# rodluger/starry_process

Measured on AMD Instinct MI355X. Metric: log_likelihood evals/sec (ydeg=15, K=1000), higher is better.
Workload: dtype f64

## Files before the change

### include/starry_process_amd.h

```cpp
#ifndef STARRY_PROCESS_AMD_H
#define STARRY_PROCESS_AMD_H

#include <stdint.h>

#ifdef __cplusplus
extern "C" {
#endif

typedef struct sp_handle sp_handle;

typedef enum {
  SP_OK = 0,
  SP_ERR_INVALID = -1,
  SP_ERR_HIP = -2,
  SP_ERR_NO_DEVICE = -3,
  SP_ERR_STATE = -4,
  SP_ERR_ALLOC = -5,
  SP_ERR_COMM = -6
} sp_status;

#define SP_STAR_NOT_PD 1u
#define SP_STAR_ZMAX 2u
#define SP_STAR_NAN 4u
#define SP_STAR_STALE_PLAN 8u
// ... 185 lines not shown
                         double *dnodes_da_host, double *dweights_da_host, double *dnodes_db_host,
                         double *dweights_db_host);

int sp_ylm_moments_quadrature(sp_handle *h, const double *vecs_host, int mv, int first_is_col,
                              const double *phi_host, const double *w_host, int P, int Q, double g,
                              double sqrt_n, double epsy, double epsy15, double *mean_dev,
                              double *cov_dev, void *stream);
int sp_ylm_moments_quadrature_grad(sp_handle *h, const double *s_host, const double *ds_dr_host,
                                   const double *phi_host, const double *w_host, const double *dphi_host,
                                   const double *dw_host, int P, int Q, double g, double sqrt_n, double epsy,
                                   double epsy15, double *mean_dev, double *cov_dev, double *dmean_dev,
                                   double *dcov_dev, void *stream);

int sp_profile_begin(sp_handle *h, int max_launches);
int sp_profile_end(sp_handle *h, long *launches, double *total_ms, double *flops);
int sp_profile_kind(sp_handle *h, int kind, long *launches, double *total_ms, double *flops);
int sp_profile_kind_ex(sp_handle *h, int kind, long *launches, double *total_ms, double *flops, double *flops_padded);
int sp_profile_begin_kinds(sp_handle *h, int max_launches, unsigned kind_mask);

int sp_set_defer_norm(sp_handle *h, int on);

int sp_set_lazy_cov(sp_handle *h, int on);

int sp_allgather_lnlike(sp_handle *h, void *nccl_comm, const double *local_dev, int count,
                        double *all_dev, void *stream);

int sp_debug_set_look_ahead(sp_handle *h, int on);
int sp_debug_set_panel_layout(sp_handle *h, int layout, int fuse_reduce);
int sp_debug_panel2_trace(long long *out);
int sp_debug_panel2_chain(long long *out);
int sp_debug_set_syrk128_from(int blocks);
int sp_debug_set_syrk_symdiag(int on);
int sp_debug_set_small_k(int on);
int sp_debug_asm_chunks(int ntr, int nchunk, int *start_host);

#ifdef __cplusplus
}
#endif
#endif
```

### starry_process_amd/_lib.py

```python
import ctypes
import os

import numpy as np

_HERE = os.path.dirname(os.path.abspath(__file__))
LIB_PATH = os.path.join(_HERE, "libsp_hip.so")
if os.environ.get("SP_LIB_VARIANT"):
    LIB_PATH = os.path.join(_HERE, "libsp_hip_%s.so" % os.environ["SP_LIB_VARIANT"])

c_double_p = ctypes.POINTER(ctypes.c_double)
c_int32_p = ctypes.POINTER(ctypes.c_int32)
c_void_p = ctypes.c_void_p


class sp_star(ctypes.Structure):

    _fields_ = [
        ("period", ctypes.c_double),
        ("inc", ctypes.c_double),
        ("tau", ctypes.c_double),
        ("baseline_var", ctypes.c_double),
        ("baseline_mean", ctypes.c_double),
        ("data_var", ctypes.c_double),
        ("table", ctypes.c_int32),
# ... 58 lines not shown
    "sp_ylm_conditional_workspace_bytes": (ctypes.c_size_t, [_V, _I, _I]),
    "sp_ylm_conditional_batched": (_I, [_V, _I, _I, _V, _V, _V, _V, _V, _V, _V, _V, _V, _V, _V, _V, _V]),
    "sp_ylm_conditional_whitened": (_I, [_V, _I, _I, _V, _V, _V, _V, _V, _V, _V, _V, _V, _V]),
    "sp_alpha_beta": (_I, [_D, _I, c_double_p, c_double_p, c_double_p, c_double_p]),
    "sp_set_marginal_constants": (_I, [_V, _V, _V]),
    "sp_set_ylm_moments": (_I, [_V, _V, _V]),
    "sp_set_ylm_moments_dev": (_I, [_V, _V, _V, _V]),
    "sp_get_polar_moments": (_I, [_V, _V, _V]),
    "sp_ylm_moments_quadrature": (_I, [_V, _V, _I, _I, _V, _V, _I, _I, _D, _D, _D, _D,
                                       _V, _V, _V]),
    "sp_ylm_moments_quadrature_grad": (_I, [_V, _V, _V, _V, _V, _V, _V, _I, _I, _D, _D, _D, _D,
                                            _V, _V, _V, _V, _V]),
    "sp_debug_panel2_trace": (_I, [_V]),
    "sp_debug_panel2_chain": (_I, [_V]),
    "sp_debug_asm_chunks": (_I, [_I, _I, _V]),
    "sp_debug_set_syrk128_from": (_I, [_I]),
    "sp_debug_set_small_k": (_I, [_I]),
    "sp_debug_set_syrk_symdiag": (_I, [_I]),
    "sp_debug_set_look_ahead": (_I, [_V, _I]),
    "sp_debug_set_panel_layout": (_I, [_V, _I, _I]),
    "sp_profile_kind": (_I, [_V, _I, ctypes.POINTER(ctypes.c_long), c_double_p, c_double_p]),
    "sp_profile_kind_ex": (_I, [_V, _I, ctypes.POINTER(ctypes.c_long), c_double_p, c_double_p, c_double_p]),
    "sp_set_lazy_cov": (_I, [_V, _I]),
    "sp_set_defer_norm": (_I, [_V, _I]),
    "sp_profile_begin_kinds": (_I, [_V, _I, ctypes.c_uint]),
    "sp_profile_begin": (_I, [_V, _I]),
    "sp_profile_end": (_I, [_V, ctypes.POINTER(ctypes.c_long), c_double_p, c_double_p]),
    "sp_kernel_table": (_I, [_V, _V, _I, _I, _V, _V, _V, _V]),
    "sp_cov_marginal_batched": (
        _I, [_V, _I, _I, _V, _V, _I, _V, _V, _I, _I, _I, _V, _L, _L, _V, _V]),
    "sp_design_matrix": (_I, [_V, _I, _I, _V, _V, _V, _V, _V]),
    "sp_cov_conditional_batched": (
        _I, [_V, _I, _I, _V, _V, _V, _I, _I, _I, _V, _L, _L, _V, _V, _V]),
    "sp_cho_factor": (_I, [_V, _V, _I, _L, _L, _I, _V, _V]),
    "sp_cho_solve": (_I, [_V, _V, _I, _L, _L, _V, _I, _I, _V]),
    "sp_tri_solve": (_I, [_V, _V, _I, _L, _L, _V, _I, _I, _I, _V]),
    "sp_solve_rev": (_I, [_V, _V, _I, _L, _L, _V, _V, _I, _I, _I, _V, _V, _V]),
    "sp_cholesky_rev": (_I, [_V, _V, _I, _L, _L, _V, _I, _V, _V]),
    "sp_lnlike_workspace_bytes": (_L, [_V, _I, _I, _I]),
    "sp_lnlike_ensemble": (
        _I, [_V, _I, _I, _I, _V, _V, _V, _V, _I, _I, _V, _V, _V, _I, _I, _I, _D,
             _V, _V, _V, _V]),
    "sp_cholesky_lnlike_batched": (_I, [_V, _I, _I, _I, _V, _V, _V, _V, _V, _V]),
    "sp_plan_data": (_I, [_V, _I, _I, _I, _V, _V, _V, _V, _I, _I, _V, _V, ctypes.POINTER(_V)]),
    "sp_plan_destroy": (None, [_V]),
    "sp_plan_replicate": (_I, [_V, _V, _I, _V, ctypes.POINTER(_V)]),
# ... 76 lines not shown
```

### starry_process_amd/csrc/sp_api.hip

```cpp
#include <algorithm>
#include <cmath>
#include <cstdio>
#include <cstdlib>
#include <dlfcn.h>
#include <cstring>
#include <new>

#include "sp_internal.h"
#include "sp_cov.h"

int sp_launch_kernel_table(sp_handle *h, const double *rta1_dev, int ntab,
                           int covpts, const double *xp_dev, double *tab_dev,
                           double *meanvar_dev, hipStream_t st, int nsets = 0, const double *ez_dev = nullptr,
                           const double *Ez_dev = nullptr);
int sp_launch_theta(int S, int K, const double *t, const sp_star *stars,
                    double *theta, hipStream_t st, int32_t *info = nullptr,
                    uint32_t *status = nullptr, const double *tab = nullptr, int covpts = 0,
                    double *ptab = nullptr);
int sp_launch_spline_index(int K, const double *theta, double dx, long long *out,
                           hipStream_t st);
int sp_launch_rowsum(int S, int K, const double *theta, const double *t,
                     const sp_star *stars, int covpts, const double *tab,
                     const double *meanvar, const double *xp, int temporal,
                     const double *raw, double *rowsum, hipStream_t st);
// ... 11 lines not shown
                       int lazy_nfull = 0);
int sp_launch_assemble_sums(int S, int K, int M, int Kp, const double *theta, const double *t,
                            const sp_star *stars, int covpts, const double *ptab, const double *meanvar,
                            int temporal, const double *flux, double *sys, hipStream_t st, double *part,
                            int lazy_nfull, int *nflat);
int sp_launch_defer_finish(int S, int K, int M, int Kp, const sp_star *stars, const double *meanvar,
                           const double *condmean, int order, double zmax, const double *part,
                           const double *diag, const double *flux, double *sys, void *coef, double *rscal,
                           uint32_t *status, hipStream_t st, int nflat = 0);
int sp_launch_assemble_planned(int S, int K, int M, int Kp, const PlanDev &plan, const double *t,
                               const sp_star *stars, int covpts, const double *tab, const double *meanvar,
                               int temporal, const double *flux, const double *diag, double *sys, int nfull,
                               int ncolw, int order, double zmax, void *coef, double *rscal, double *ptab, int32_t *info,
                               uint32_t *status, hipStream_t st, double *img, long lts, int fuse0, double *rid, int dfrom);
int sp_launch_cholesky_systems(sp_handle *h, double *sys, int S, int K, int Kp,
                               int32_t *info, double *invL, hipStream_t st);
bool sp_small_k_serves(int K, int M, int covpts, bool has_diag);
static int g_small_k = -1;
static bool sp_small_k_on() {
  if (g_small_k >= 0) return g_small_k != 0;
  static const bool env = !(getenv("SP_SMALL_K") && atoi(getenv("SP_SMALL_K")) == 0);
  return env;
}
int sp_launch_small_lnlike(int S, int K, int M, const PlanDev &plan, const double *t, const sp_star *stars, int covpts,
                           const double *tab, const double *meanvar, int temporal, const double *flux, const double *diag,
                           int order, double zmax, double *lnlike, uint32_t *status_out, hipStream_t st);
int sp_launch_cond_system(const double *B1, const double *A, int N, int Kr, int S, int K, int M, int Kp,
                          const double *t, const sp_star *stars, int temporal, const void *coef,
                          const double *diag, const double *flux, double *sys, double *part,
                          hipStream_t st);
int sp_launch_cholesky_groups(sp_handle *h, int ngroups, const sp_chol_group *grp, int K,
                              int Kp);
int sp_launch_lnlike_reduce(const double *sys, int S, int K, int M, int Kp,
                            const int32_t *info, double *lnlike, uint32_t *status,
                            hipStream_t st, uint32_t *status_out = nullptr,
                            const sp_star *stars = nullptr, const void *defer_coef = nullptr,
                            const double *rscal = nullptr, int dvec = 0);
int sp_launch_pad_in(const double *A, int K, long lda, long strideA, double *sys,
                     int Kp, int M, const double *resid, int S, hipStream_t st, int ident = 0,
                     int32_t *nonfinite = nullptr);
int sp_launch_pad_out(const double *sys, int Kp, double *A, int K, long lda,
                      long strideA, const int32_t *info, int S, hipStream_t st);
int sp_launch_cho_solve(const double *L, int K, long ldl, long strideL, double *B,
                        int nrhs, int batch, hipStream_t st);
int sp_launch_ylm_gram(int S, int K, int N, const double *A, const double *flux, const double *diag,
                       const sp_star *stars, int whitened, const double *sinv, const double *sinvmu, double *Bt,
// ... 716 lines not shown
    ms += dt;
    fl += h->prof_fl[i / 2];
    flp += h->prof_flp[i / 2];
    n += h->prof_n[i / 2];
  }
  if (launches) *launches = n;
  if (total_ms) *total_ms = ms;
  if (flops) *flops = fl;
  if (flops_padded) *flops_padded = flp;
  return SP_OK;
}

int sp_profile_end(sp_handle *h, long *launches, double *total_ms, double *flops) {
  return sp_profile_kind(h, SP_PROF_SYRK, launches, total_ms, flops);
}

int sp_set_lazy_cov(sp_handle *h, int on) {
  if (h && h->device < 0) return SP_ERR_NO_DEVICE;
  if (!h) return SP_ERR_INVALID;
  h->lazy_cov = on ? 1 : 0;
  return SP_OK;
}

int sp_set_defer_norm(sp_handle *h, int on) {
  if (h && h->device < 0) return SP_ERR_NO_DEVICE;
  if (!h || (on != 0 && on != 1)) return SP_ERR_INVALID;
  h->defer_norm = on;
  return SP_OK;
}

int sp_debug_set_small_k(int on) {
  g_small_k = on < 0 ? -1 : (on ? 1 : 0);
  return SP_OK;
}

int sp_debug_set_look_ahead(sp_handle *h, int on) {
  if (!h) return SP_ERR_INVALID;
  h->look_ahead = on ? 1 : 0;
  return SP_OK;
}

int sp_debug_set_panel_layout(sp_handle *h, int layout, int fuse_reduce) {
  if (!h) return SP_ERR_INVALID;
  h->panel_layout = layout ? 1 : 0;
  h->fuse_reduce = fuse_reduce ? 1 : 0;
  return SP_OK;
// ... 356 lines not shown

int sp_lnlike_ensemble_planned(sp_handle *h, const sp_plan *plan, const double *t_dev, const double *flux_dev,
                               const double *diag_dev, const sp_star *stars_dev, const double *tab_dev,
                               const double *meanvar_dev, int norm_order, double zmax, void *workspace_dev,
                               double *lnlike_dev, uint32_t *status_dev, void *stream) {
  if (h && h->device < 0) return SP_ERR_NO_DEVICE;
  if (!h || !plan || !stars_dev || !tab_dev || !meanvar_dev || !workspace_dev || !lnlike_dev ||
      norm_order < 0 || norm_order > SP_NORM_MAXORDER)
    return SP_ERR_INVALID;
  if (plan->device != h->device) return SP_ERR_INVALID;
  if (!t_dev && !flux_dev && !diag_dev) {
    t_dev = plan->t;
    flux_dev = plan->flux;
    diag_dev = plan->diag;
  } else if (t_dev != plan->t || flux_dev != plan->flux || diag_dev != plan->diag) {
    return SP_ERR_INVALID;
  }
  const int S = plan->S, K = plan->K, M = plan->M, covpts = plan->covpts, temporal = plan->temporal;
  if (h->xp_covpts != covpts) return SP_ERR_STATE;
  hipStream_t st = (hipStream_t)stream;
  if (sp_small_k_on() && sp_small_k_serves(K, M, covpts, diag_dev != nullptr))
    return sp_launch_small_lnlike(S, K, M, plan->dev, t_dev, stars_dev, covpts, tab_dev, meanvar_dev, temporal, flux_dev,
                                  diag_dev, norm_order, zmax, lnlike_dev, status_dev, st);
  Layout L = make_layout(h, S, K, M, true);
  void *ws = workspace_dev;
  double *ptab = 4 * (size_t)(covpts + 4) > (size_t)L.Kr * L.N ? nullptr : at<double>(ws, L.A);
  int lazy_nfull = 0, ncolw = 0, no_panels = 0;
  static const bool riding_env = !(getenv("SP_PLAN_RIDING_LAZY") && atoi(getenv("SP_PLAN_RIDING_LAZY")) == 0);
  bool riding = false;
  const int nrid = M + (diag_dev ? 2 : 1);
  double *rid = at<double>(ws, L.B1);
  if (h->lazy_cov && ptab && K / SP_NB >= 2 && 4 * (covpts + 4) + 64 <= SP_TILE_LDS_MIN) {
    riding = riding_env && ((size_t)nrid + 1) * K <= (size_t)L.Kr * L.N;
    lazy_nfull = riding ? L.Kp / SP_NB : K / SP_NB;
    static const bool panel_lazy = !(getenv("SP_PLAN_PANEL_LAZY") && atoi(getenv("SP_PLAN_PANEL_LAZY")) == 0);
    if (temporal != SP_TEMPORAL_NONE || !panel_lazy) {
      static const bool tl = !(getenv("SP_PLAN_TEMPORAL_LAZY") && atoi(getenv("SP_PLAN_TEMPORAL_LAZY")) == 0);
      ncolw = sp_superpanel_width(h, K);
      no_panels = 1;
      if ((!tl && temporal != SP_TEMPORAL_NONE) || ncolw * SP_NB >= K) lazy_nfull = ncolw = no_panels = 0;
    }
  }
  static const bool dlazy_env = !(getenv("SP_PLAN_DIAG_LAZY") && atoi(getenv("SP_PLAN_DIAG_LAZY")) == 0);
  const int ntr = L.Kp / SP_NB, wsp = sp_superpanel_width(h, K), nsteps = (K + SP_NB - 1) / SP_NB;
  int dlazy = 0, dfrom = ntr;
  if (dlazy_env && riding && lazy_nfull == ntr && wsp * SP_NB < K && sp_syrk_can_form_diag(ntr - wsp) &&
// ... 1 lines not shown
    const int last = wsp < nsteps - 1 ? wsp : nsteps - 1;
    dlazy = 2;
    dfrom = last + 1;
  }
  static const bool fuse0_env = !(getenv("SP_PLAN_FUSE0") && atoi(getenv("SP_PLAN_FUSE0")) == 0);
  const int fuse0 = (fuse0_env && K >= SP_NB) ? 1 : 0;
  int rc = sp_launch_assemble_planned(S, K, M, L.Kp, plan->dev, t_dev, stars_dev, covpts, tab_dev, meanvar_dev, temporal,
                                      flux_dev, diag_dev, at<double>(ws, L.sys), lazy_nfull, ncolw, norm_order, zmax,
                                      at<double>(ws, L.coef), at<double>(ws, L.rscal), ptab, at<int32_t>(ws, L.info),
                                      at<uint32_t>(ws, L.status), st, at<double>(ws, L.invL), sp_lt_stride(L.Kp), fuse0,
                                      riding ? rid : nullptr, dfrom);
  if (rc) return rc;
  const bool fused_reduce = sp_panel_fuses_reduce(h, K, L.Kp);
  sp_chol_group G{at<double>(ws, L.sys), at<int32_t>(ws, L.info), at<double>(ws, L.invL), S, st, LazyCov{}, SpReduceArgs{}};
  if (fused_reduce)
    G.red = SpReduceArgs{lnlike_dev, at<uint32_t>(ws, L.status), status_dev, stars_dev, (const void *)at<double>(ws, L.coef),
                         at<double>(ws, L.rscal), diag_dev ? 1 : 0, K, M, K + M + (diag_dev ? 2 : 1)};
  G.block0_done = fuse0 != 0;
  (void)dlazy;
  if (lazy_nfull)
    G.lazy = LazyCov{plan->dev.theta, t_dev, stars_dev, ptab, K, covpts, temporal, lazy_nfull, 0, 0, no_panels ? 0 : 1,
                     no_panels, riding ? rid : nullptr, riding ? nrid : 0, dlazy, plan->dev.inorder};
  if ((rc = sp_launch_cholesky_groups(h, 1, &G, K, L.Kp))) return rc;
  if (!fused_reduce) return lnlike_finish(L, ws, K, M, lnlike_dev, status_dev, st, stars_dev, true, diag_dev != nullptr);
  return SP_OK;
}

int sp_gemm_nt(sp_handle *h, const double *A_dev, long lda, long strideA, const double *B_dev,
               long ldb, long strideB, double *C_dev, long ldc, long strideC, int M, int N,
               int K, double alpha, int beta, int lower_only, int batch, void *stream) {
  if (h && h->device < 0) return SP_ERR_NO_DEVICE;
  if (!h || !A_dev || !B_dev || !C_dev || M < 0 || N < 0 || K < 0 || batch < 0 || lda < K ||
      ldb < K || ldc < N || (beta != 0 && beta != 1))
    return SP_ERR_INVALID;
  return sp_launch_gemm_nt(A_dev, lda, strideA, B_dev, ldb, strideB, C_dev, ldc, strideC, M, N, K,
                           alpha, beta, lower_only, batch, (hipStream_t)stream);
}

int sp_gp_condition(sp_handle *h, int K, int Ks, const double *Ktt_dev, const double *Kst_dev,
                    double *Kss_dev, const double *r_dev, double *mu_dev, int32_t *info_dev,
                    void *stream) {
  if (h && h->device < 0) return SP_ERR_NO_DEVICE;
  if (!h || K < 1 || Ks < 1 || !Ktt_dev || !Kst_dev || !Kss_dev || !r_dev || !mu_dev)
    return SP_ERR_INVALID;
  hipStream_t st = (hipStream_t)stream;
  const int M = Ks + 1, Kp = sp_roundup(K + M, SP_NB);
  SpCarve c;
  const size_t osys = c.take(sizeof(double) * (size_t)Kp * Kp), ores = c.take(sizeof(double) * (size_t)M * K),
// ... 293 lines not shown
```

### starry_process_amd/csrc/sp_host.cpp

```cpp
#include <cmath>
#include <cstring>

#include "sp_internal.h"

namespace {

inline int nidx(int l, int m) { return l * l + l + m; }

inline void mono_mul_acc(double *acc, int l1, int m1, int l2, int m2, double v) {
  const bool z1 = ((l1 + m1) & 1) != 0, z2 = ((l2 + m2) & 1) != 0;
  const int l = l1 + l2, m = m1 + m2;
  if (z1 && z2) {
    acc[nidx(l - 2, m)] += v;
    acc[nidx(l, m - 2)] += -v;
    acc[nidx(l, m + 2)] += -v;
  } else {
    acc[nidx(l, m)] += v;
  }
}

void times_z(int deg, const double *p, double *out, int nout) {
  for (int i = 0; i < nout; ++i) out[i] = 0.0;
  for (int l = 0; l <= deg; ++l)
    for (int m = -l; m <= l; ++m) {
// ... 293 lines not shown
  return SP_OK;
}

int sp_alpha_beta(double z, int order, double *alpha, double *beta,
                  double *dalpha_dz, double *dbeta_dz) {
  if (order < 0) return SP_ERR_INVALID;
  double fac = 1.0, a = 0.0, b = 0.0, da = 0.0, db = 0.0, df = 0.0;
  for (int n = 0; n <= order; ++n) {
    da += df;
    db += 2 * n * df;
    df = (2 * n + 3) * (df * z + fac);
    a += fac;
    b += 2 * n * fac;
    fac *= z * (2 * n + 3);
  }
  if (alpha) *alpha = a;
  if (beta) *beta = b;
  if (dalpha_dz) *dalpha_dz = da;
  if (dbeta_dz) *dbeta_dz = db;
  return SP_OK;
}

int sp_version(void) { return 100; }

const char *sp_strerror(int status) {
  switch (status) {
    case SP_OK: return "ok";
    case SP_ERR_INVALID: return "invalid argument";
    case SP_ERR_HIP: return "HIP runtime error";
    case SP_ERR_NO_DEVICE: return "no usable gfx950 device";
    case SP_ERR_STATE: return "constants or Ylm moments not set";
    case SP_ERR_ALLOC: return "allocation failed";
    case SP_ERR_COMM: return "RCCL not loaded in this process, or the collective failed";
    default: return "unknown status";
  }
}

}

namespace {

double hyp2f1_series(double a, double b, double c, double z) {
  double term = a * b * z / c;
  double dtermdb = a * z / c, dtermdc = -term / c;
  double value = 1.0 + term, dfdb = dtermdb, dfdc = dtermdc;
  int n = 1;
// ... 227 lines not shown
```

### starry_process_amd/csrc/sp_internal.h

```cpp
#ifndef SP_INTERNAL_H
#define SP_INTERNAL_H

#include <hip/hip_runtime.h>
#include <stdint.h>
#include <vector>

#include "../../include/starry_process_amd.h"

#define SP_WAVE 64
#define SP_MAX_YDEG 30
#define SP_MAX_UDEG 4
#define SP_NORM_MAXORDER 64

#define SP_NB 64

struct SpScratch {
  void *ptr = nullptr;
  size_t bytes = 0;
};

struct sp_handle {
  int ydeg = 0, udeg = 0, N = 0, NWIG = 0, device = 0;
  std::vector<int32_t> l_of, m_of, mirror, m0, blk;
  std::vector<double> rT;
// ... 20 lines not shown
  SpScratch tab_scratch;
  bool table_attr_done = false;
  SpScratch big;
  struct CsSlot {
    double *host = nullptr;
    double *dev = nullptr;
    size_t cap = 0;
    hipEvent_t done = nullptr;
    bool used = false;
  };
  std::vector<CsSlot> cs_ring;
  int cs_next = 0;
  int superpanel = 0;
  int groups = 1;
  int ncu = 256;
  int look_ahead = 1;
  int panel_layout = 1;
  int fuse_reduce = 1;
  std::vector<hipStream_t> gstream;
  std::vector<hipEvent_t> gdone;
  hipEvent_t gfork = nullptr;
  int defer_norm = 1;
  int lazy_cov = 1;
  bool prof_on = false;
  unsigned prof_mask = 1u;
  std::vector<hipEvent_t> prof_ev;
  std::vector<int> prof_kind;
  std::vector<double> prof_fl;
  std::vector<double> prof_flp;
  std::vector<int> prof_n;
  size_t prof_used = 0;
};

enum {
  SP_PROF_SYRK = 0, SP_PROF_CHAIN = 2, SP_PROF_PANELS = 4, SP_PROF_PANEL_LAUNCH = 5, SP_PROF_NKINDS = 6
};

struct SpProfScope {
  sp_handle *h;
  hipStream_t st;
  bool on;
  size_t idx;
  SpProfScope(sp_handle *h_, hipStream_t st_, int kind, double flops, int launches = 1, double flops_padded = -1.0)
      : h(h_), st(st_), on(false), idx(0) {
    if (!h || !h->prof_on || !((h->prof_mask >> kind) & 1u) || h->prof_used + 2 > h->prof_ev.size()) return;
    idx = h->prof_used;
    h->prof_used += 2;
    h->prof_kind[idx / 2] = kind;
    h->prof_fl[idx / 2] = flops;
    h->prof_flp[idx / 2] = flops_padded < 0.0 ? flops : flops_padded;
    h->prof_n[idx / 2] = launches;
    if (hipEventRecord(h->prof_ev[idx], st) != hipSuccess) {
      h->prof_n[idx / 2] = 0;
      h->prof_fl[idx / 2] = 0.0;
      h->prof_flp[idx / 2] = 0.0;
      h->prof_kind[idx / 2] = -1;
      return;
    }
// ... 83 lines not shown
  int tr0, tc0;
  int c0lazy;
  int no_panels;
  const double *rid;
  int nrid;
  int dlazy;
  const double *inorder;
};

int sp_syrk_can_form_diag(int nb);

struct SpCoef {
  double c1;
  double zab;
  double za;
  double z;
  double gpmean;
  double m;
  double mu;
  double d1;
};
static_assert(sizeof(SpCoef) == 64, "8 doubles per star (Layout::coef)");

struct PlanDev {
  const double *theta;
  const double *wbar;
  const double *sflux;
  const double *sdv;
  const double *key;
  const double *inorder;
};
struct sp_plan {
  int device, S, K, M, covpts, temporal, has_diag;
  void *buf;
  size_t bytes;
  PlanDev dev;
  const double *t, *flux, *diag;
  int nrep;
};

#define SP_RSCAL_HEAD 3
struct SpReduceArgs {
  double *lnlike;
  uint32_t *status, *status_out;
  const sp_star *stars;
  const void *coef;
  const double *rscal;
  int dvec;
  int K, M;
  int live_rows;
};

struct sp_chol_group {
  double *sys;
  int32_t *info;
  double *invL;
  int S;
  hipStream_t st;
  LazyCov lazy;
  SpReduceArgs red;
  int tri0 = -1;
// ... 57 lines not shown
```

### starry_process_amd/csrc/sp_plan.hip

```cpp
#include <new>

#include "sp_internal.h"
#include "sp_cov.h"

int sp_launch_theta(int S, int K, const double *t, const sp_star *stars, double *theta, hipStream_t st,
                    int32_t *info = nullptr, uint32_t *status = nullptr, const double *tab = nullptr,
                    int covpts = 0, double *ptab = nullptr);

namespace {

template <int TK>
__global__ __launch_bounds__(256) void plan_wbar_kernel(
    int K, const double *__restrict__ theta, const double *__restrict__ t, const sp_star *__restrict__ stars,
    int covpts, double *__restrict__ partial) {
  extern __shared__ __attribute__((aligned(16))) double bins[];
  const int s = blockIdx.y, np = covpts + 4, tid = threadIdx.x, wave = tid >> 6;
  for (int k = tid; k < 4 * np; k += 256) bins[k] = 0.0;
  __syncthreads();
  const int tile = blockIdx.x;
  int ta = (int)((sqrtf(8.0f * tile + 1.0f) - 1.0f) * 0.5f);
  while (ta * (ta + 1) / 2 > tile) --ta;
  while ((ta + 1) * (ta + 2) / 2 <= tile) ++ta;
  const int tb = tile - ta * (ta + 1) / 2;
  const int i = tb * 64 + (tid & 63);
// ... 31 lines not shown
  __syncthreads();
  double *P = partial + ((size_t)s * gridDim.x + blockIdx.x) * np;
  for (int k = tid; k < np; k += 256) P[k] = (bins[k] + bins[np + k]) + (bins[2 * np + k] + bins[3 * np + k]);
}

__global__ __launch_bounds__(256) void plan_wbar_reduce_kernel(int np, int nwg, const double *__restrict__ partial,
                                                               double *__restrict__ wbar) {
  __shared__ double red[4][64];
  const int s = blockIdx.y, k = blockIdx.x * 64 + (threadIdx.x & 63), g = threadIdx.x >> 6;
  double a = 0.0;
  if (k < np) {
#pragma unroll 4
    for (int w = g; w < nwg; w += 4) a += partial[((size_t)s * nwg + w) * np + k];
  }
  red[g][threadIdx.x & 63] = a;
  __syncthreads();
  if (g == 0 && k < np)
    wbar[(size_t)s * np + k] = (red[0][threadIdx.x] + red[1][threadIdx.x]) + (red[2][threadIdx.x] + red[3][threadIdx.x]);
}

__global__ __launch_bounds__(256) void plan_scalars_kernel(
    int K, int M, const double *__restrict__ flux, const double *__restrict__ diag,
    const sp_star *__restrict__ stars, const double *__restrict__ t, double *__restrict__ sflux,
    double *__restrict__ sdv, double *__restrict__ key, double *__restrict__ inorder) {
  __shared__ double red[4];
  const int s = blockIdx.x, tid = threadIdx.x;
  const sp_star st = stars[s];
  const int nobs = star_nobs(st, K);
  auto block_sum = [&](double v) {
    for (int off = 32; off > 0; off >>= 1) v += __shfl_down(v, off, 64);
    __syncthreads();
    if ((tid & 63) == 0) red[tid >> 6] = v;
    __syncthreads();
    return (red[0] + red[1]) + (red[2] + red[3]);
  };
  for (int m = 0; m <= M; ++m) {
    const double *src = m < M ? flux + ((size_t)s * M + m) * K : (diag ? diag + (size_t)s * K : nullptr);
    double a = 0.0;
    if (src)
      for (int i = tid; i < nobs; i += 256) a += src[i];
    const double total = block_sum(a);
    if (tid == 0) {
      if (m < M) sflux[(size_t)s * M + m] = total;
      else sdv[s] = total;
    }
  }
  int unsorted = 0;
  for (int i = tid; i + 1 < nobs; i += 256)
    if (!(t[(size_t)s * K + i + 1] >= t[(size_t)s * K + i])) unsorted = 1;
  unsorted = __syncthreads_or(unsorted);
  if (tid == 0) {
    inorder[s] = unsorted ? 0.0 : 1.0;
    key[3 * s] = st.period;
    key[3 * s + 1] = st.tau;
    key[3 * s + 2] = (double)nobs;
  }
}

}

extern "C" {

int sp_plan_data(sp_handle *h, int S, int K, int M, const double *t_dev, const double *flux_dev,
                 const double *diag_dev, const sp_star *stars_dev, int covpts, int temporal, void *workspace_dev,
                 void *stream, sp_plan **out) {
  if (h && h->device < 0) return SP_ERR_NO_DEVICE;
  if (!h || !out || !t_dev || !flux_dev || !stars_dev || !workspace_dev || S < 1 || K < 2 || M < 1 || covpts < 1)
    return SP_ERR_INVALID;
  if (temporal != SP_TEMPORAL_NONE && temporal != SP_TEMPORAL_MATERN32 && temporal != SP_TEMPORAL_EXPSQUARED)
    return SP_ERR_INVALID;
  *out = nullptr;
  hipStream_t st = (hipStream_t)stream;
  const int np = covpts + 4;
  const int ntr = (K + 63) / 64, ntl = ntr * (ntr + 1) / 2;
  const long ws_bytes = sp_lnlike_workspace_bytes(h, S, K, M);
  const size_t Kp = (size_t)sp_roundup(K + M, SP_NB);
  if (ws_bytes < 0 || (size_t)ntl * np > Kp * Kp) return SP_ERR_INVALID;
  const size_t lds = sizeof(double) * 4 * (size_t)np;
  if (lds > 150 * 1024) return SP_ERR_INVALID;
  double *partial = reinterpret_cast<double *>(static_cast<char *>(workspace_dev) + (size_t)ws_bytes) - (size_t)S * Kp * Kp;

  SP_HIP(hipSetDevice(h->device));
  sp_plan *p = new (std::nothrow) sp_plan();
  if (!p) return SP_ERR_ALLOC;
  p->device = h->device;
  p->S = S; p->K = K; p->M = M; p->covpts = covpts; p->temporal = temporal; p->has_diag = diag_dev != nullptr;
  p->t = t_dev; p->flux = flux_dev; p->diag = diag_dev; p->nrep = 0;
  const size_t d = sizeof(double);
  SpCarve c;
  const size_t o_theta = c.take(d * S * K), o_wbar = c.take(d * S * np), o_sflux = c.take(d * S * M),
               o_sdv = c.take(d * S), o_key = c.take(d * S * 3), o_ord = c.take(d * S);
  p->bytes = c.off;
  hipError_t e = hipMalloc(&p->buf, c.off);
  if (e != hipSuccess) {
    sp_set_hip_error(e, "hipMalloc(plan)");
    delete p;
    return SP_ERR_ALLOC;
  }
  double *theta = at<double>(p->buf, o_theta), *wbar = at<double>(p->buf, o_wbar);
  double *sflux = at<double>(p->buf, o_sflux), *sdv = at<double>(p->buf, o_sdv);
  double *key = at<double>(p->buf, o_key), *inorder = at<double>(p->buf, o_ord);
  p->dev = PlanDev{theta, wbar, sflux, sdv, key, inorder};
  auto fail = [&](int rc) {
    (void)hipFree(p->buf);
    delete p;
    return rc;
  };
  int rc = sp_launch_theta(S, K, t_dev, stars_dev, theta, st);
  if (rc) return fail(rc);
  hipLaunchKernelGGL(plan_scalars_kernel, dim3(S), dim3(256), 0, st, K, M, flux_dev, diag_dev, stars_dev, t_dev, sflux,
                     sdv, key, inorder);
  dim3 grid(ntl, S);
#define SP_PLAN_WBAR(TK)                                                                                          \
  do {                                                                                                            \
    (void)hipFuncSetAttribute(reinterpret_cast<const void *>(plan_wbar_kernel<TK>),                               \
                              hipFuncAttributeMaxDynamicSharedMemorySize, 150 * 1024);                            \
    hipLaunchKernelGGL((plan_wbar_kernel<TK>), grid, dim3(256), lds, st, K, theta, t_dev, stars_dev, covpts, partial); \
  } while (0)
  if (temporal == SP_TEMPORAL_NONE) SP_PLAN_WBAR(SP_TEMPORAL_NONE);
  else if (temporal == SP_TEMPORAL_MATERN32) SP_PLAN_WBAR(SP_TEMPORAL_MATERN32);
  else SP_PLAN_WBAR(SP_TEMPORAL_EXPSQUARED);
#undef SP_PLAN_WBAR
  hipLaunchKernelGGL(plan_wbar_reduce_kernel, dim3((np + 63) / 64, S), dim3(256), 0, st, np, ntl, partial, wbar);
  e = hipGetLastError();
  if (e != hipSuccess) {
    sp_set_hip_error(e, "kernel launch (plan)");
    return fail(SP_ERR_HIP);
  }
  e = hipStreamSynchronize(st);
  if (e != hipSuccess) {
    sp_set_hip_error(e, "hipStreamSynchronize(plan)");
    return fail(SP_ERR_HIP);
  }
  *out = p;
  return SP_OK;
}

namespace {
__global__ __launch_bounds__(256) void replicate_kernel(const double *__restrict__ src, long n, double *__restrict__ dst) {
  const long i = (long)blockIdx.x * 256 + threadIdx.x;
  if (i < n) dst[(size_t)blockIdx.y * n + i] = src[i];
}
}

int sp_plan_replicate(sp_handle *h, const sp_plan *src, int B, void *stream, sp_plan **out) {
  if (h && h->device < 0) return SP_ERR_NO_DEVICE;
  if (!h || !src || !out || B < 1 || B > 65535 || src->device != h->device || (long)src->S * B > (1L << 24))
    return SP_ERR_INVALID;
  *out = nullptr;
  hipStream_t st = (hipStream_t)stream;
  SP_HIP(hipSetDevice(h->device));
  sp_plan *p = new (std::nothrow) sp_plan(*src);
  if (!p) return SP_ERR_ALLOC;
  const int S0 = src->S, K = src->K, M = src->M, np = src->covpts + 4;
  p->S = S0 * B;
  p->nrep = B;
  p->buf = nullptr;
  const size_t d = sizeof(double), S = (size_t)p->S;
  SpCarve c;
  const size_t o_theta = c.take(d * S * K), o_wbar = c.take(d * S * np), o_sflux = c.take(d * S * M),
               o_sdv = c.take(d * S), o_key = c.take(d * S * 3), o_ord = c.take(d * S), o_t = c.take(d * S * K),
               o_flux = c.take(d * S * M * K), o_diag = src->has_diag ? c.take(d * S * K) : c.off;
  p->bytes = c.off;
  hipError_t e = hipMalloc(&p->buf, c.off);
  if (e != hipSuccess) {
    sp_set_hip_error(e, "hipMalloc(plan replica)");
    delete p;
    return SP_ERR_ALLOC;
  }
  void *buf = p->buf;
  p->dev = PlanDev{at<double>(buf, o_theta), at<double>(buf, o_wbar), at<double>(buf, o_sflux),
                   at<double>(buf, o_sdv), at<double>(buf, o_key), at<double>(buf, o_ord)};
  p->t = at<double>(buf, o_t);
  p->flux = at<double>(buf, o_flux);
  p->diag = src->has_diag ? at<double>(buf, o_diag) : nullptr;
  auto rep = [&](const double *from, size_t n, double *to) {
    hipLaunchKernelGGL(replicate_kernel, dim3((unsigned)((n + 255) / 256), B), dim3(256), 0, st, from, (long)n, to);
  };
  rep(src->dev.theta, (size_t)S0 * K, at<double>(buf, o_theta));
  rep(src->dev.wbar, (size_t)S0 * np, at<double>(buf, o_wbar));
  rep(src->dev.sflux, (size_t)S0 * M, at<double>(buf, o_sflux));
  rep(src->dev.sdv, (size_t)S0, at<double>(buf, o_sdv));
  rep(src->dev.key, (size_t)S0 * 3, at<double>(buf, o_key));
  rep(src->dev.inorder, (size_t)S0, at<double>(buf, o_ord));
  rep(src->t, (size_t)S0 * K, at<double>(buf, o_t));
  rep(src->flux, (size_t)S0 * M * K, at<double>(buf, o_flux));
  if (src->has_diag) rep(src->diag, (size_t)S0 * K, at<double>(buf, o_diag));
  e = hipGetLastError();
  if (e == hipSuccess) e = hipStreamSynchronize(st);
  if (e != hipSuccess) {
    sp_set_hip_error(e, "sp_plan_replicate");
    (void)hipFree(p->buf);
    delete p;
    return SP_ERR_HIP;
  }
  *out = p;
  return SP_OK;
}

int sp_plan_systems(const sp_plan *plan) { return plan ? plan->S : SP_ERR_INVALID; }

void sp_plan_destroy(sp_plan *plan) {
  if (!plan) return;
  if (plan->buf) (void)hipFree(plan->buf);
  delete plan;
}

// ... 9 lines not shown
```

### starry_process_amd/engine.py

```python
import ctypes
import os

import numpy as np

from . import _lib
from . import hostconst
from ._lib import STAR_DTYPE, TEMPORAL, SPError, c_void_p, check, hptr

__all__ = ["Engine", "DataPlan", "get_engine", "make_stars", "stars_for_samples", "sample_parameters", "samples_in_bounds"]


def _torch():
    import torch

    return torch


def make_stars(S, period=1.0, inc_deg=60.0, tau=0.0, baseline_var=0.0,
               baseline_mean=0.0, data_var=0.0, table=0, nobs=0):
    st = np.zeros(S, dtype=STAR_DTYPE)
    st["period"] = period
    st["inc"] = np.asarray(inc_deg, dtype=float) * (np.pi / 180)
    st["tau"] = tau
    st["baseline_var"] = baseline_var
# ... 391 lines not shown
        info = torch.zeros(B, dtype=torch.int32, device=self.device)
        check(self._L.sp_spd_inverse_batched(self._h, B, K, self._p(Cb), K, K * K, self._p(out), self._p(logdet),
                                             self._p(info), self._p(ws), self._stream()))
        if not full:
            return out, logdet, info
        low = torch.tril(out[:, :K, :K])
        inv = low + torch.tril(low, -1).transpose(1, 2)
        return (inv if C.dim() == 3 else inv[0]), (logdet if C.dim() == 3 else logdet[0]), info

    def cho_solve(self, L, b):
        L = self.f64(L)
        b = self.f64(b).clone()
        Lb = L if L.dim() == 3 else L.unsqueeze(0)
        B, K, _ = Lb.shape
        shape = b.shape
        bb = b.reshape(B, K, -1).contiguous()
        nrhs = bb.shape[2]
        check(self._L.sp_cho_solve(self._h, self._p(Lb), K, K, K * K, self._p(bb), nrhs, B, self._stream()))
        return bb.reshape(shape)

    def set_lazy_cov(self, on):
        check(self._L.sp_set_lazy_cov(self._h, int(bool(on))))

    def set_defer_norm(self, on):
        check(self._L.sp_set_defer_norm(self._h, int(bool(on))))
        self._ws = None

    def tri_solve(self, L, b, trans=False):
        L = self.f64(L)
        b = self.f64(b).clone()
        Lb = L if L.dim() == 3 else L.unsqueeze(0)
        B, K, _ = Lb.shape
        shape = b.shape
        bb = b.reshape(B, K, -1).contiguous()
        check(self._L.sp_tri_solve(self._h, self._p(Lb), K, K, K * K, self._p(bb), bb.shape[2], B,
                                   int(bool(trans)), self._stream()))
        return bb.reshape(shape)

    def solve_rev(self, L, c, c_bar, trans=False):
        L = self.f64(L)
        Lb = (L if L.dim() == 3 else L.unsqueeze(0)).contiguous()
        B, K, _ = Lb.shape
        c = self.f64(c)
        shape = c.shape
        cb = c.reshape(B, K, -1).contiguous()
        gb = self.f64(c_bar).reshape(B, K, -1).contiguous()
# ... 227 lines not shown
```

Before: 106,600.

## Add Toeplitz Schur factorization path for uniformly sampled light curves

Plan construction now flags each star whose observation times are sorted, lie on a uniform grid, do not wrap a rotation period and have no per-point diagonal. For those stars the log-likelihood runs a new kernel that factorizes the stationary (Toeplitz) covariance with a generalized Schur recursion in registers. It also performs the forward solves for the flux columns in the same kernel. This replaces the dense O(K^3) Cholesky with O(K^2) work, one block per star. When only some stars qualify, the dense path still runs for all of them and the Toeplitz kernel then overwrites the flagged ones, which adds redundant work in mixed batches.

Result: no change. 106,600, median of 6 (-0.1%).

```diff
diff --git a/include/starry_process_amd.h b/include/starry_process_amd.h
--- a/include/starry_process_amd.h
+++ b/include/starry_process_amd.h
@@ -231,6 +231,9 @@
 
 int sp_set_lazy_cov(sp_handle *h, int on);
 
+int sp_set_toeplitz(sp_handle *h, int on);
+int sp_toeplitz_classify(const double *t_host, int nobs, double period, int has_diag);
+
 int sp_allgather_lnlike(sp_handle *h, void *nccl_comm, const double *local_dev, int count,
                         double *all_dev, void *stream);
 
diff --git a/starry_process_amd/_lib.py b/starry_process_amd/_lib.py
--- a/starry_process_amd/_lib.py
+++ b/starry_process_amd/_lib.py
@@ -104,6 +104,8 @@
     "sp_profile_kind": (_I, [_V, _I, ctypes.POINTER(ctypes.c_long), c_double_p, c_double_p]),
     "sp_profile_kind_ex": (_I, [_V, _I, ctypes.POINTER(ctypes.c_long), c_double_p, c_double_p, c_double_p]),
     "sp_set_lazy_cov": (_I, [_V, _I]),
+    "sp_set_toeplitz": (_I, [_V, _I]),
+    "sp_toeplitz_classify": (_I, [_V, _I, ctypes.c_double, _I]),
     "sp_set_defer_norm": (_I, [_V, _I]),
     "sp_profile_begin_kinds": (_I, [_V, _I, ctypes.c_uint]),
     "sp_profile_begin": (_I, [_V, _I]),
diff --git a/starry_process_amd/csrc/sp_api.hip b/starry_process_amd/csrc/sp_api.hip
--- a/starry_process_amd/csrc/sp_api.hip
+++ b/starry_process_amd/csrc/sp_api.hip
@@ -57,6 +57,10 @@
   static const bool env = !(getenv("SP_SMALL_K") && atoi(getenv("SP_SMALL_K")) == 0);
   return env;
 }
+bool sp_toeplitz_serves(int K, int M, int covpts, bool has_diag);
+int sp_launch_toeplitz_lnlike(int S, int K, int M, const PlanDev &plan, const double *t, const sp_star *stars,
+                              int covpts, const double *tab, const double *meanvar, int temporal, const double *flux,
+                              int order, double zmax, double *lnlike, uint32_t *status_out, hipStream_t st);
 int sp_launch_small_lnlike(int S, int K, int M, const PlanDev &plan, const double *t, const sp_star *stars, int covpts,
                            const double *tab, const double *meanvar, int temporal, const double *flux, const double *diag,
                            int order, double zmax, double *lnlike, uint32_t *status_out, hipStream_t st);
@@ -819,6 +823,13 @@
   return SP_OK;
 }
 
+int sp_set_toeplitz(sp_handle *h, int on) {
+  if (h && h->device < 0) return SP_ERR_NO_DEVICE;
+  if (!h) return SP_ERR_INVALID;
+  h->toeplitz = on ? 1 : 0;
+  return SP_OK;
+}
+
 int sp_set_defer_norm(sp_handle *h, int on) {
   if (h && h->device < 0) return SP_ERR_NO_DEVICE;
   if (!h || (on != 0 && on != 1)) return SP_ERR_INVALID;
@@ -1221,6 +1232,13 @@
   if (sp_small_k_on() && sp_small_k_serves(K, M, covpts, diag_dev != nullptr))
     return sp_launch_small_lnlike(S, K, M, plan->dev, t_dev, stars_dev, covpts, tab_dev, meanvar_dev, temporal, flux_dev,
                                   diag_dev, norm_order, zmax, lnlike_dev, status_dev, st);
+  const bool toep = h->toeplitz && plan->ntoep > 0 && sp_toeplitz_serves(K, M, covpts, diag_dev != nullptr);
+  auto launch_toep = [&]() {
+    SpProfScope prof(h, st, SP_PROF_TOEPLITZ, (double)plan->ntoep * (4.0 + 2.0 * (M + 1)) * 0.5 * K * (K + 1.0));
+    return sp_launch_toeplitz_lnlike(S, K, M, plan->dev, t_dev, stars_dev, covpts, tab_dev, meanvar_dev, temporal,
+                                     flux_dev, norm_order, zmax, lnlike_dev, status_dev, st);
+  };
+  if (toep && plan->ntoep == S) return launch_toep();
   Layout L = make_layout(h, S, K, M, true);
   void *ws = workspace_dev;
   double *ptab = 4 * (size_t)(covpts + 4) > (size_t)L.Kr * L.N ? nullptr : at<double>(ws, L.A);
@@ -1268,8 +1286,9 @@
     G.lazy = LazyCov{plan->dev.theta, t_dev, stars_dev, ptab, K, covpts, temporal, lazy_nfull, 0, 0, no_panels ? 0 : 1,
                      no_panels, riding ? rid : nullptr, riding ? nrid : 0, dlazy, plan->dev.inorder};
   if ((rc = sp_launch_cholesky_groups(h, 1, &G, K, L.Kp))) return rc;
-  if (!fused_reduce) return lnlike_finish(L, ws, K, M, lnlike_dev, status_dev, st, stars_dev, true, diag_dev != nullptr);
-  return SP_OK;
+  if (!fused_reduce && (rc = lnlike_finish(L, ws, K, M, lnlike_dev, status_dev, st, stars_dev, true, diag_dev != nullptr)))
+    return rc;
+  return toep ? launch_toep() : SP_OK;
 }
 
 int sp_gemm_nt(sp_handle *h, const double *A_dev, long lda, long strideA, const double *B_dev,
diff --git a/starry_process_amd/csrc/sp_host.cpp b/starry_process_amd/csrc/sp_host.cpp
--- a/starry_process_amd/csrc/sp_host.cpp
+++ b/starry_process_amd/csrc/sp_host.cpp
@@ -339,6 +339,16 @@
 }
 
 int sp_version(void) { return 100; }
+
+int sp_toeplitz_classify(const double *t_host, int nobs, double period, int has_diag) {
+  if (!t_host || nobs < 1) return SP_ERR_INVALID;
+  if (has_diag || nobs <= SP_TOEPLITZ_MIN_K || !sp_toeplitz_no_wrap(t_host[0], t_host[nobs - 1], period)) return 0;
+  for (int i = 0; i + 1 < nobs; ++i)
+    if (!(t_host[i + 1] >= t_host[i])) return 0;
+  for (int i = 0; i < nobs; ++i)
+    if (!sp_toeplitz_on_grid(t_host[i], t_host[0], t_host[nobs - 1], i, nobs)) return 0;
+  return 1;
+}
 
 const char *sp_strerror(int status) {
   switch (status) {
diff --git a/starry_process_amd/csrc/sp_internal.h b/starry_process_amd/csrc/sp_internal.h
--- a/starry_process_amd/csrc/sp_internal.h
+++ b/starry_process_amd/csrc/sp_internal.h
@@ -66,6 +66,7 @@
   hipEvent_t gfork = nullptr;
   int defer_norm = 1;
   int lazy_cov = 1;
+  int toeplitz = 1;
   bool prof_on = false;
   unsigned prof_mask = 1u;
   std::vector<hipEvent_t> prof_ev;
@@ -77,7 +78,7 @@
 };
 
 enum {
-  SP_PROF_SYRK = 0, SP_PROF_CHAIN = 2, SP_PROF_PANELS = 4, SP_PROF_PANEL_LAUNCH = 5, SP_PROF_NKINDS = 6
+  SP_PROF_SYRK = 0, SP_PROF_CHAIN = 2, SP_PROF_PANELS = 4, SP_PROF_PANEL_LAUNCH = 5, SP_PROF_TOEPLITZ = 6, SP_PROF_NKINDS = 7
 };
 
 struct SpProfScope {
@@ -207,6 +208,15 @@
 };
 static_assert(sizeof(SpCoef) == 64, "8 doubles per star (Layout::coef)");
 
+#define SP_TOEPLITZ_MIN_K 128
+__host__ __device__ inline bool sp_toeplitz_on_grid(double ti, double t0, double tn, int i, int n) {
+  const double span = tn - t0, dt = span / (double)(n - 1);
+  return span > 0.0 && fabs(ti - t0 - (double)i * dt) <= 8.0 * 2.220446049250313e-16 * fabs(span);
+}
+__host__ __device__ inline bool sp_toeplitz_no_wrap(double t0, double tn, double period) {
+  return period > 0.0 && floor(t0 / period) == floor(tn / period);
+}
+
 struct PlanDev {
   const double *theta;
   const double *wbar;
@@ -214,6 +224,7 @@
   const double *sdv;
   const double *key;
   const double *inorder;
+  const double *toep;
 };
 struct sp_plan {
   int device, S, K, M, covpts, temporal, has_diag;
@@ -222,6 +233,7 @@
   PlanDev dev;
   const double *t, *flux, *diag;
   int nrep;
+  int ntoep;
 };
 
 #define SP_RSCAL_HEAD 3
diff --git a/starry_process_amd/csrc/sp_plan.hip b/starry_process_amd/csrc/sp_plan.hip
--- a/starry_process_amd/csrc/sp_plan.hip
+++ b/starry_process_amd/csrc/sp_plan.hip
@@ -1,4 +1,5 @@
 #include <new>
+#include <vector>
 
 #include "sp_internal.h"
 #include "sp_cov.h"
@@ -77,7 +78,7 @@
 __global__ __launch_bounds__(256) void plan_scalars_kernel(
     int K, int M, const double *__restrict__ flux, const double *__restrict__ diag,
     const sp_star *__restrict__ stars, const double *__restrict__ t, double *__restrict__ sflux,
-    double *__restrict__ sdv, double *__restrict__ key, double *__restrict__ inorder) {
+    double *__restrict__ sdv, double *__restrict__ key, double *__restrict__ inorder, double *__restrict__ toep) {
   __shared__ double red[4];
   const int s = blockIdx.x, tid = threadIdx.x;
   const sp_star st = stars[s];
@@ -100,12 +101,18 @@
       else sdv[s] = total;
     }
   }
-  int unsorted = 0;
+  int unsorted = 0, offgrid = 0;
+  const double *ts = t + (size_t)s * K;
   for (int i = tid; i + 1 < nobs; i += 256)
-    if (!(t[(size_t)s * K + i + 1] >= t[(size_t)s * K + i])) unsorted = 1;
+    if (!(ts[i + 1] >= ts[i])) unsorted = 1;
+  for (int i = tid; i < nobs; i += 256)
+    if (!sp_toeplitz_on_grid(ts[i], ts[0], ts[nobs - 1], i, nobs)) offgrid = 1;
   unsorted = __syncthreads_or(unsorted);
+  offgrid = __syncthreads_or(offgrid);
   if (tid == 0) {
     inorder[s] = unsorted ? 0.0 : 1.0;
+    toep[s] = (!diag && nobs > SP_TOEPLITZ_MIN_K && !unsorted && !offgrid &&
+               sp_toeplitz_no_wrap(ts[0], ts[nobs - 1], st.period)) ? 1.0 : 0.0;
     key[3 * s] = st.period;
     key[3 * s + 1] = st.tau;
     key[3 * s + 2] = (double)nobs;
@@ -144,7 +151,7 @@
   const size_t d = sizeof(double);
   SpCarve c;
   const size_t o_theta = c.take(d * S * K), o_wbar = c.take(d * S * np), o_sflux = c.take(d * S * M),
-               o_sdv = c.take(d * S), o_key = c.take(d * S * 3), o_ord = c.take(d * S);
+               o_sdv = c.take(d * S), o_key = c.take(d * S * 3), o_ord = c.take(d * S), o_toep = c.take(d * S);
   p->bytes = c.off;
   hipError_t e = hipMalloc(&p->buf, c.off);
   if (e != hipSuccess) {
@@ -154,8 +161,8 @@
   }
   double *theta = at<double>(p->buf, o_theta), *wbar = at<double>(p->buf, o_wbar);
   double *sflux = at<double>(p->buf, o_sflux), *sdv = at<double>(p->buf, o_sdv);
-  double *key = at<double>(p->buf, o_key), *inorder = at<double>(p->buf, o_ord);
-  p->dev = PlanDev{theta, wbar, sflux, sdv, key, inorder};
+  double *key = at<double>(p->buf, o_key), *inorder = at<double>(p->buf, o_ord), *toep = at<double>(p->buf, o_toep);
+  p->dev = PlanDev{theta, wbar, sflux, sdv, key, inorder, toep};
   auto fail = [&](int rc) {
     (void)hipFree(p->buf);
     delete p;
@@ -164,7 +171,7 @@
   int rc = sp_launch_theta(S, K, t_dev, stars_dev, theta, st);
   if (rc) return fail(rc);
   hipLaunchKernelGGL(plan_scalars_kernel, dim3(S), dim3(256), 0, st, K, M, flux_dev, diag_dev, stars_dev, t_dev, sflux,
-                     sdv, key, inorder);
+                     sdv, key, inorder, toep);
   dim3 grid(ntl, S);
 #define SP_PLAN_WBAR(TK)                                                                                          \
   do {                                                                                                            \
@@ -186,6 +193,16 @@
   if (e != hipSuccess) {
     sp_set_hip_error(e, "hipStreamSynchronize(plan)");
     return fail(SP_ERR_HIP);
+  }
+  {
+    std::vector<double> fl(S);
+    e = hipMemcpy(fl.data(), toep, sizeof(double) * S, hipMemcpyDeviceToHost);
+    if (e != hipSuccess) {
+      sp_set_hip_error(e, "hipMemcpy(plan flags)");
+      return fail(SP_ERR_HIP);
+    }
+    p->ntoep = 0;
+    for (int i = 0; i < S; ++i) p->ntoep += fl[i] != 0.0;
   }
   *out = p;
   return SP_OK;
@@ -214,7 +231,8 @@
   const size_t d = sizeof(double), S = (size_t)p->S;
   SpCarve c;
   const size_t o_theta = c.take(d * S * K), o_wbar = c.take(d * S * np), o_sflux = c.take(d * S * M),
-               o_sdv = c.take(d * S), o_key = c.take(d * S * 3), o_ord = c.take(d * S), o_t = c.take(d * S * K),
+               o_sdv = c.take(d * S), o_key = c.take(d * S * 3), o_ord = c.take(d * S), o_toep = c.take(d * S),
+               o_t = c.take(d * S * K),
                o_flux = c.take(d * S * M * K), o_diag = src->has_diag ? c.take(d * S * K) : c.off;
   p->bytes = c.off;
   hipError_t e = hipMalloc(&p->buf, c.off);
@@ -225,7 +243,8 @@
   }
   void *buf = p->buf;
   p->dev = PlanDev{at<double>(buf, o_theta), at<double>(buf, o_wbar), at<double>(buf, o_sflux),
-                   at<double>(buf, o_sdv), at<double>(buf, o_key), at<double>(buf, o_ord)};
+                   at<double>(buf, o_sdv), at<double>(buf, o_key), at<double>(buf, o_ord), at<double>(buf, o_toep)};
+  p->ntoep = src->ntoep * B;
   p->t = at<double>(buf, o_t);
   p->flux = at<double>(buf, o_flux);
   p->diag = src->has_diag ? at<double>(buf, o_diag) : nullptr;
@@ -238,6 +257,7 @@
   rep(src->dev.sdv, (size_t)S0, at<double>(buf, o_sdv));
   rep(src->dev.key, (size_t)S0 * 3, at<double>(buf, o_key));
   rep(src->dev.inorder, (size_t)S0, at<double>(buf, o_ord));
+  rep(src->dev.toep, (size_t)S0, at<double>(buf, o_toep));
   rep(src->t, (size_t)S0 * K, at<double>(buf, o_t));
   rep(src->flux, (size_t)S0 * M * K, at<double>(buf, o_flux));
   if (src->has_diag) rep(src->diag, (size_t)S0 * K, at<double>(buf, o_diag));
diff --git a/starry_process_amd/csrc/sp_toeplitz.hip b/starry_process_amd/csrc/sp_toeplitz.hip
--- /dev/null
+++ b/starry_process_amd/csrc/sp_toeplitz.hip
@@ -0,0 +1,251 @@
+#include "sp_internal.h"
+#include "sp_cov.h"
+#include "sp_asm.h"
+#include "sp_reduce.h"
+
+namespace {
+
+typedef SpCoef Coef;
+
+struct ToepSrc {
+  const double *dg;
+  const double *rows;
+  int ldr;
+  __device__ __forceinline__ double diag(int i) const { return dg[i]; }
+  __device__ __forceinline__ double row(int m, int k) const { return rows[m * ldr + k]; }
+};
+
+__device__ __forceinline__ double tp_read_lane(double v, int l) {
+  const int lo = __builtin_amdgcn_readlane(__double2loint(v), l);
+  const int hi = __builtin_amdgcn_readlane(__double2hiint(v), l);
+  return __hiloint2double(hi, lo);
+}
+__device__ __forceinline__ double tp_shr1(double v) {
+  const int lo = __builtin_amdgcn_update_dpp(0, __double2loint(v), 0x138, 0xf, 0xf, false);
+  const int hi = __builtin_amdgcn_update_dpp(0, __double2hiint(v), 0x138, 0xf, 0xf, false);
+  return __hiloint2double(hi, lo);
+}
+
+constexpr int TP_BCW = 8;
+constexpr int TP_MAXW = 4;
+
+template <int NS, int MR, int TK>
+__global__ __launch_bounds__(256) void toeplitz_lnlike_kernel(
+    int K, int M, PlanDev plan, const double *__restrict__ t, const sp_star *__restrict__ stars, int covpts,
+    const double *__restrict__ tab, const double *__restrict__ meanvar, const double *__restrict__ flux, int order,
+    double zmax, double *__restrict__ lnlike, uint32_t *__restrict__ status_out) {
+  extern __shared__ __attribute__((aligned(16))) double lds[];
+  const int s = blockIdx.x;
+  if (plan.toep[s] == 0.0) return;
+  const int tid = threadIdx.x, W = blockDim.x >> 6, lane = tid & 63, wave = tid >> 6, np = covpts + 4;
+  double *sTab = lds;
+  double *sDg = sTab + 4 * np;
+  double *sY = sDg + K;
+  double *sRed = sY + MR * K;
+  double *sBc = sRed + 48;
+  double *sX = sBc + 2 * TP_BCW;
+  double *sRs = sX + 2 * TP_MAXW;
+  Coef *sCoef = reinterpret_cast<Coef *>(sRs + SP_RSCAL_HEAD + M + ((SP_RSCAL_HEAD + M) & 1));
+  uint32_t *sStat = reinterpret_cast<uint32_t *>(reinterpret_cast<double *>(sCoef) + 8);
+  const sp_star st = stars[s];
+  const int nobs = star_nobs(st, K);
+  const double *th = plan.theta + (size_t)s * K, *tt = t + (size_t)s * K;
+  double dot = 0.0;
+  {
+    const double *src = tab + (size_t)st.table * 5 * np, *wb = plan.wbar + (size_t)s * np;
+    for (int e = tid; e < np; e += blockDim.x) {
+      *reinterpret_cast<dd2 *>(sTab + 2 * e) = dd2{src[np + e], src[2 * np + e]};
+      *reinterpret_cast<dd2 *>(sTab + 2 * np + 2 * e) = dd2{src[3 * np + e], src[4 * np + e]};
+    }
+    if (wave == 0)
+      for (int e = lane; e < np; e += 64) dot += src[e] * wb[e];
+  }
+  for (int e = tid; e < (MR + 1) * K; e += blockDim.x) sDg[e] = e < K ? 1.0 : 0.0;
+  for (int off = 32; off > 0; off >>= 1) dot += __shfl_down(dot, off, 64);
+  if (tid == 0) sRed[0] = dot;
+  __syncthreads();
+  const double fmean = meanvar[2 * st.table];
+  const double m = sRed[0] / ((double)nobs * (double)nobs);
+  const Coef c = defer_coef(m, fmean, order, st.baseline_var);
+  const double inv_c1 = 1.0 / c.c1;
+  if (tid == 0) {
+    const double delta = st.data_var / c.c1;
+    sRs[0] = (double)nobs * m;
+    sRs[1] = (double)nobs * delta;
+    sRs[2] = delta;
+    *sCoef = c;
+    const double *key = plan.key + 3 * (size_t)s;
+    const bool stale = !(key[0] == st.period) || (TK != SP_TEMPORAL_NONE && !(key[1] == st.tau)) || key[2] != (double)nobs;
+    *sStat = (c.z > zmax ? SP_STAR_ZMAX : 0u) | (stale ? SP_STAR_STALE_PLAN : 0u);
+  }
+  for (int mm = tid; mm < M; mm += blockDim.x)
+    sRs[SP_RSCAL_HEAD + mm] = plan.sflux[(size_t)s * M + mm] - (double)nobs * st.baseline_mean;
+  SplineGen g{sTab, 2 * np, 6.283185307179586 / covpts, 1.0 / (6.283185307179586 / covpts), covpts};
+  const int i0 = tid * NS;
+  const double th0 = th[0], t0 = TK != SP_TEMPORAL_NONE ? tt[0] : 0.0;
+  double U[NS], V[NS], B[MR][NS];
+  double c00;
+  {
+#pragma clang fp contract(off)
+    c00 = g(th0, th0) * temporal_factor(TK, t0, t0, st.tau) + st.data_var * inv_c1;
+  }
+  const double sq = sqrt(c00);
+#pragma unroll
+  for (int q0 = 0; q0 < NS; q0 += 4) {
+    double a[4], b[4], o[4];
+#pragma unroll
+    for (int e = 0; e < 4; ++e) {
+      const int i = i0 + q0 + e;
+      a[e] = i < nobs ? th[i] : th0;
+      b[e] = th0;
+    }
+    g.many<4>(a, b, o);
+#pragma unroll
+    for (int e = 0; e < 4; ++e) {
+      const int i = i0 + q0 + e;
+      double cv = 0.0;
+      if (i < nobs) {
+#pragma clang fp contract(off)
+        cv = o[e] * temporal_factor(TK, tt[i], t0, st.tau);
+        if (i == 0) cv = c00;
+      }
+      U[q0 + e] = cv / sq;
+      V[q0 + e] = i == 0 ? 0.0 : cv / sq;
+    }
+  }
+#pragma unroll
+  for (int mr = 0; mr < MR; ++mr)
+#pragma unroll
+    for (int q = 0; q < NS; ++q) {
+      const int i = i0 + q;
+      double v = 0.0;
+      if (i < nobs) v = mr < M ? flux[((size_t)s * M + mr) * K + i] - st.baseline_mean : 1.0;
+      B[mr][q] = v;
+    }
+  int notpd = !(c00 > 0.0);
+  for (int jb = 0; jb < nobs && !notpd; jb += NS) {
+    const int ob = jb / NS;
+#pragma unroll
+    for (int q = 0; q < NS; ++q) {
+      const int j = jb + q;
+      const int o1 = q + 1 < NS ? ob : ob + 1;
+      const bool live = j < nobs && !notpd, more = j + 1 < nobs;
+      double Ljj = 1.0, bj[MR], vj1 = 0.0, xin = 0.0;
+#pragma unroll
+      for (int mr = 0; mr < MR; ++mr) bj[mr] = 0.0;
+      if (W == 1) {
+        if (live) {
+          Ljj = tp_read_lane(U[0], ob);
+#pragma unroll
+          for (int mr = 0; mr < MR; ++mr) bj[mr] = tp_read_lane(B[mr][q], ob);
+          vj1 = tp_read_lane(V[(q + 1) % NS], more ? o1 : ob);
+        }
+      } else if (live) {
+        double *bc = sBc + (j & 1) * TP_BCW, *xf = sX + (j & 1) * TP_MAXW;
+        if (tid == ob) {
+          bc[0] = U[0];
+#pragma unroll
+          for (int mr = 0; mr < MR; ++mr) bc[1 + mr] = B[mr][q];
+        }
+        if (tid == o1) bc[1 + MR] = V[(q + 1) % NS];
+        if (lane == 63) xf[wave] = U[NS - 1 - q];
+        __syncthreads();
+        Ljj = bc[0];
+#pragma unroll
+        for (int mr = 0; mr < MR; ++mr) bj[mr] = bc[1 + mr];
+        vj1 = bc[1 + MR];
+        if (wave > 0) xin = xf[wave - 1];
+      }
+      if (!more) vj1 = 0.0;
+      const double inv = 1.0 / Ljj;
+      const double rho = vj1 * inv;
+      if (live && (!(Ljj > 0.0) || !(fabs(rho) < 1.0))) notpd = 1;
+      if (live && !notpd) {
+        double y[MR];
+#pragma unroll
+        for (int mr = 0; mr < MR; ++mr) y[mr] = bj[mr] * inv;
+        if (tid == ob) {
+          sDg[j] = Ljj;
+#pragma unroll
+          for (int mr = 0; mr < MR; ++mr) sY[mr * K + j] = y[mr];
+        }
+#pragma unroll
+        for (int r = 0; r < NS; ++r) {
+          const double l = U[(r - q + NS) % NS];
+#pragma unroll
+          for (int mr = 0; mr < MR; ++mr) B[mr][r] = fma(-y[mr], l, B[mr][r]);
+        }
+        if (more) {
+          double sh = tp_shr1(U[NS - 1 - q]);
+          if (W > 1 && lane == 0) sh = xin;
+          U[NS - 1 - q] = sh;
+          const double sg = sqrt((1.0 - rho) * (1.0 + rho)), isg = 1.0 / sg;
+#pragma unroll
+          for (int r = 0; r < NS; ++r) {
+            const int p = (r - q - 1 + 2 * NS) % NS;
+            const double un = fma(-rho, V[r], U[p]) * isg;
+            V[r] = fma(-rho, un, sg * V[r]);
+            U[p] = un;
+          }
+        }
+      }
+    }
+  }
+  notpd = __syncthreads_or(notpd);
+  if (notpd && tid == 0) sDg[0] = __builtin_nan("");
+  __syncthreads();
+  if (tid >= 64) return;
+  lnlike_reduce_src<false, ToepSrc, 64, 4>(ToepSrc{sDg, sY, K}, nobs, M, nullptr, lnlike + s, sStat,
+                                           status_out ? status_out + s : nullptr, stars + s, sCoef, sRs, 0, sRed, tid,
+                                           notpd);
+}
+
+int tp_ns(int K) { return K <= 256 ? 4 : (K <= 512 ? 8 : 16); }
+
+size_t tp_lds_bytes(int K, int M, int covpts) {
+  return sizeof(double) * (4 * (size_t)(covpts + 4) + (size_t)(M + 2) * K + 48 + 2 * TP_BCW + 2 * TP_MAXW +
+                           SP_RSCAL_HEAD + M + 1 + 8 + 2);
+}
+
+}
+
+bool sp_toeplitz_serves(int K, int M, int covpts, bool has_diag) {
+  if (has_diag || M < 1 || M + 1 > 4 || K <= SP_TOEPLITZ_MIN_K || K > 64 * 16 * TP_MAXW) return false;
+  return tp_lds_bytes(K, M, covpts) <= 150 * 1024;
+}
+
+int sp_launch_toeplitz_lnlike(int S, int K, int M, const PlanDev &plan, const double *t, const sp_star *stars,
+                              int covpts, const double *tab, const double *meanvar, int temporal, const double *flux,
+                              int order, double zmax, double *lnlike, uint32_t *status_out, hipStream_t st) {
+  if (!sp_toeplitz_serves(K, M, covpts, false) || !plan.toep) return SP_ERR_INVALID;
+  const int NS = tp_ns(K), W = (K + 64 * NS - 1) / (64 * NS);
+  const size_t lds = tp_lds_bytes(K, M, covpts);
+#define SP_TOEP(NSV, MRV, TKV)                                                                                       \
+  do {                                                                                                               \
+    (void)hipFuncSetAttribute(reinterpret_cast<const void *>(toeplitz_lnlike_kernel<NSV, MRV, TKV>),                 \
+                              hipFuncAttributeMaxDynamicSharedMemorySize, 150 * 1024);                               \
+    hipLaunchKernelGGL((toeplitz_lnlike_kernel<NSV, MRV, TKV>), dim3(S), dim3(64 * W), lds, st, K, M, plan, t, stars, \
+                       covpts, tab, meanvar, flux, order, zmax, lnlike, status_out);                                 \
+  } while (0)
+#define SP_TOEP_TK(NSV, MRV)                                                              \
+  do {                                                                                    \
+    if (temporal == SP_TEMPORAL_NONE) SP_TOEP(NSV, MRV, SP_TEMPORAL_NONE);                \
+    else if (temporal == SP_TEMPORAL_MATERN32) SP_TOEP(NSV, MRV, SP_TEMPORAL_MATERN32);   \
+    else if (temporal == SP_TEMPORAL_EXPSQUARED) SP_TOEP(NSV, MRV, SP_TEMPORAL_EXPSQUARED); \
+    else return SP_ERR_INVALID;                                                           \
+  } while (0)
+#define SP_TOEP_MR(NSV)                    \
+  do {                                     \
+    if (M == 1) SP_TOEP_TK(NSV, 2);        \
+    else if (M == 2) SP_TOEP_TK(NSV, 3);   \
+    else SP_TOEP_TK(NSV, 4);               \
+  } while (0)
+  if (NS == 4) SP_TOEP_MR(4);
+  else if (NS == 8) SP_TOEP_MR(8);
+  else SP_TOEP_MR(16);
+#undef SP_TOEP_MR
+#undef SP_TOEP_TK
+#undef SP_TOEP
+  SP_LAUNCH_CHECK();
+  return SP_OK;
+}
diff --git a/starry_process_amd/engine.py b/starry_process_amd/engine.py
--- a/starry_process_amd/engine.py
+++ b/starry_process_amd/engine.py
@@ -437,6 +437,9 @@
     def set_lazy_cov(self, on):
         check(self._L.sp_set_lazy_cov(self._h, int(bool(on))))
 
+    def set_toeplitz(self, on):
+        check(self._L.sp_set_toeplitz(self._h, int(bool(on))))
+
     def set_defer_norm(self, on):
         check(self._L.sp_set_defer_norm(self._h, int(bool(on))))
         self._ws = None
```
